# RicoFio/disentangle_mlp

Measured on AMD Instinct MI355X. Metric: celeba64_betavaegan_train_images_per_sec, higher is better.
Workload: dtype fp32-equivalent (fp16x3 split of fp32 operands on the f16 MFMA, fp32 accumulate, every convolution and the Linear layers with >= 2^20 weights (vg_gemm_nt_f16x3); the small Linear layers (vendor GEMMs), BatchNorm, losses, Adam in fp32)

## Files before the change

### disentangle_mlp_amd/_lib.py

```python
import ctypes
import os
from ctypes import c_float, c_int, c_size_t, c_void_p

import torch

_HERE = os.path.dirname(os.path.abspath(__file__))
LIB_PATH = os.path.join(_HERE, "libvaegan_hip.so")
ABI_VERSION = 7

_P, _I, _F, _Z = c_void_p, c_int, c_float, c_size_t

SIGNATURES = {
    "vg_version": (_I, []),
    "vg_conv5x5_fwd": (_I, [_P, _P, _P, _P, _I, _I, _I, _I, _I, _I, _P]),
    "vg_convT5x5_fwd": (_I, [_P, _P, _P, _P, _I, _I, _I, _I, _I, _I, _P]),
    "vg_conv5x5_packed_floats": (_Z, [_I, _I]),
    "vg_conv5x5_pack": (_I, [_P, _P, _I, _I, _I, _I, _P]),
    "vg_conv5x5_fwd_packed": (_I, [_P, _P, _P, _P, _I, _I, _I, _I, _I, _I, _P]),
    "vg_convT5x5_fwd_packed": (_I, [_P, _P, _P, _P, _I, _I, _I, _I, _I, _I, _P]),
    "vg_conv5x5_fwd_packed_stats_floats": (_Z, [_I, _I, _I, _I, _I, _I]),
    "vg_conv5x5_fwd_packed_stats": (_I, [_P, _P, _P, _P, _I, _I, _I, _I, _I, _I, _P, _Z, _P]),
    "vg_conv5x5_packed_bf16split_bytes": (_Z, [_I, _I, _I]),
    "vg_conv5x5_pack_bf16split": (_I, [_P, _P, _I, _I, _I, _I, _I, _P, _P]),
    "vg_gemm_nt_f16x3_workspace_bytes": (_Z, [_I, _I, _I]),
# ... 6 lines not shown
    "vg_conv_general_pack": (_I, [_P, _P, _I, _I, _I, _I, _P, _P]),
    "vg_conv_general_fwd": (_I, [_P, _P, _P, _P] + [_I] * 11 + [ctypes.c_long, _I, _P, _P, _P]),
    "vg_absmax": (_I, [_P, _Z, _P, _P]),
    "vg_absmax_affine": (_I, [_P, _P, _P, _I, _I, _I, _I, _P, _P]),
    "vg_absmax_multi": (_I, [_P, _I, _P]),
    "vg_conv5x5_pack_bf16split_multi": (_I, [_P, _I, _I, _P]),
    "vg_convT5x5_fwd_bf16split_workspace_bytes": (_Z, [_I, _I, _I, _I, _I, _I, _I]),
    "vg_convT5x5_fwd_bf16split": (_I, [_P, _P, _P, _P, _I, _I, _I, _I, _I, _I, _I, _P, _Z, _P, _P]),
    "vg_conv5x5_fwd_bf16split_workspace_bytes": (_Z, [_I, _I, _I, _I, _I, _I, _I]),
    "vg_conv5x5_bf16split_fusable": (_I, [_I, _I, _I, _I]),
    "vg_conv5x5_fwd_bf16split_stats_floats": (_Z, [_I, _I, _I, _I, _I, _I, _I]),
    "vg_convT5x5_fwd_bf16split_stats_floats": (_Z, [_I, _I, _I, _I, _I, _I, _I]),
    "vg_convT5x5_s1_thin_bf16split_ok": (_I, [_I, _I, _I, _I]),
    "vg_conv5x5_thin_wgrad_bf16split_workspace_bytes": (_Z, [_I, _I, _I, _I, _I, _I, _I]),
    "vg_conv5x5_thin_wgrad_bf16split": (_I, [_P, _P, _P, _I, _I, _I, _I, _I, _I, _I, _P, _Z, _P, _P, _I, _I, _P]),
    "vg_conv5x5_thin_bf16split_ok": (_I, [_I, _I, _I, _I, _I]),
    "vg_conv5x5_thin_bf16split_stats_floats": (_Z, [_I, _I, _I, _I, _I, _I]),
    "vg_conv5x5_thin_bf16split": (_I, [_P, _P, _P, _P, _I, _I, _I, _I, _I, _I, _I, _P, _Z, _P]),
    "vg_convT5x5_s1_thin_bf16split": (_I, [_P, _P, _P, _P, _I, _I, _I, _I, _I, _I, _P, _P, _I, _P]),
    "vg_conv5x5_fwd_bf16split": (_I, [_P, _P, _P, _P, _I, _I, _I, _I, _I, _I, _I, _P, _Z, _P, _P]),
    "vg_conv5x5_wgrad_bf16split_workspace_bytes": (_Z, [_I, _I, _I, _I, _I, _I, _I]),
    "vg_conv5x5_wgrad_bf16split": (_I, [_P, _P, _P, _I, _I, _I, _I, _I, _I, _I, _P, _Z, _P, _P, _I, _I, _P, _P, _I, _P]),
    "vg_conv5x5_wgrad_workspace_bytes": (_Z, [_I, _I, _I, _I, _I, _I]),
    "vg_conv5x5_wgrad": (_I, [_P, _P, _P, _I, _I, _I, _I, _I, _I, _P, _Z, _I, _P]),
    "vg_channel_sum": (_I, [_P, _P, _I, _I, _I, _P, _Z, _P]),
    "vg_bn_workspace_bytes": (_Z, [_I]),
    "vg_bn_act_fwd": (_I, [_P, _P, _P, _P, _P, _P, _P, _P, _I, _I, _I, _F, _F, _I, _P, _P, _Z, _P]),
    "vg_bn_act_bwd": (_I, [_P, _P, _P, _P, _P, _P, _P, _P, _P, _I, _I, _I, _I, _I, _P, _P, _Z, _P]),
    "vg_bn_finalize_stats": (_I, [_P, _I, _I, ctypes.c_double, _P, _P, _P, _P, _P, _P, _P, _P, _F, _F, _P, _P, _Z, _P]),
    "vg_bn_stats": (_I, [_P, _P, _P, _P, _P, _P, _P, _P, _P, _I, _I, _I, _F, _F, _P, _P, _Z, _P]),
    "vg_affine_act": (_I, [_P, _P, _P, _P, _I, _I, _I, _I, _P, _P]),
    "vg_bn_eval_coeffs": (_I, [_P, _P, _P, _P, _P, _P, _P, _I, _F, _I, _P, _I, ctypes.c_double, _P, _P]),
    "vg_bn_eval_act_bwd": (_I, [_P, _P, _P, _P, _P, _P, _P, _P, _P, _I, _I, _I, _I, _I, _P, _P, _Z, _P]),
    "vg_bias_act_fwd": (_I, [_P, _P, _P, _I, _I, _I, _I, _P]),
    "vg_act_bwd": (_I, [_P, _P, _P, _Z, _I, _P, _P]),
    "vg_reparam_kl_fwd": (_I, [_P, _P, _P, _P, _P, _P, _I, _I, _F, _P]),
    "vg_reparam_kl_bwd": (_I, [_P, _P, _P, _P, _P, _F, _P, _P, _I, _I, _P]),
    "vg_scale_by_scalar": (_I, [_P, _P, _P, _Z, _P]),
    "vg_sqdiff_workspace_bytes": (_Z, [_Z]),
    "vg_sqdiff_loss": (_I, [_P, _P, _P, _P, _Z, _F, _F, _P, _Z, _P]),
    "vg_bce_loss": (_I, [_P, _F, _P, _P, _I, _F, _F, _P]),
    "vg_adam_step": (_I, [_P, _I] + [ctypes.c_double] * 6 + [_P]),
    "vg_adam_prepare": (_I, [ctypes.c_double, _P, _I, ctypes.c_double, ctypes.c_double, ctypes.c_double, _P, _P]),
    "vg_adam_step_dev": (_I, [_P, _I] + [ctypes.c_double] * 3 + [_P, _P]),
    "vg_adam_step_checked": (_I, [_P, _I] + [ctypes.c_double] * 6 + [_P, _P]),
    "vg_adam_step_dev_checked": (_I, [_P, _I] + [ctypes.c_double] * 3 + [_P, _P, _P]),
    "vg_adam_step_ema": (_I, [_P, _I] + [ctypes.c_double] * 6 + [_P, _P, ctypes.c_double, _P]),
    "vg_adam_step_dev_ema": (_I, [_P, _I] + [ctypes.c_double] * 3 + [_P, _P, _P, ctypes.c_double, _P]),
    "vg_grad_sumsq_partials": (_Z, [_P, _I]),
    "vg_grad_sumsq_multi": (_I, [_P, _P, _I, _P, _Z, _P]),
    "vg_grad_clip_finalize": (_I, [_P, _Z, ctypes.c_double, _I, _P, _P]),
    "vg_adam_step_clip": (_I, [_P, _I] + [ctypes.c_double] * 6 + [_P, _P, ctypes.c_double, _P, _P]),
    "vg_adam_step_dev_clip": (_I, [_P, _I] + [ctypes.c_double] * 3 + [_P, _P, _P, ctypes.c_double, _P, _P]),
    "vg_adam_prepare_dev": (_I, [ctypes.c_double, _P, _I, _P, _I, ctypes.c_double, ctypes.c_double, _P, _P]),
    "vg_adam_step_decay": (_I, [_P, _I] + [ctypes.c_double] * 6 + [_P, _P, ctypes.c_double, _P, ctypes.c_double, _I, _P]),
    "vg_adam_step_dev_decay": (_I, [_P, _I] + [ctypes.c_double] * 3 + [_P, _P, _P, ctypes.c_double, _P, _P]),
    "vg_adam_step_dev_ema_dev": (_I, [_P, _I] + [ctypes.c_double] * 3 + [_P, _P, _P, _P, _P, _P]),
    "vg_reparam_kl_fwd_dev": (_I, [_P, _P, _P, _P, _P, _P, _I, _I, _P, _P]),
    "vg_reparam_kl_bwd_dev": (_I, [_P, _P, _P, _P, _P, _P, _P, _P, _I, _I, _P]),
    "vg_bce_loss_dev": (_I, [_P, _P, _P, _P, _I, _F, _F, _P]),
    "vg_dot_sigmoid_bce_workspace_bytes": (_Z, [_I]),
    "vg_dot_sigmoid_bce_fwd": (_I, [_P, _P, _P, _F, _P, _P, _P, _P, _I, _I, _F, _P, _Z, _P]),
    "vg_dot_sigmoid_bce_bwd": (_I, [_P, _P, _P, _P, _P, _P, _P, _I, _I, _I, _P]),
    "vg_u8_gather_normalize": (_I, [_P, _P, _P, _I, _I, _I, _I, _F, _F, _P]),
    "vg_minmax_workspace_bytes": (_Z, [_Z]),
    "vg_minmax": (_I, [_P, _Z, _P, _P, _Z, _P]),
    "vg_image_grid_shape": (_I, [_I, _I, _I, _I, _I, _P, _P]),
    "vg_image_grid_u8": (_I, [_P, _P, _P, _I, _I, _I, _I, _I, _I, _F, _P]),
    "vg_quantize_each_u8": (_I, [_P, _P, _I, _I, _I, _I, _P, _Z, _P]),
    "vg_resize_bilinear_u8": (_I, [_P, _P, _I, _I, _I, _I, _I, _F, _F, _P, _P]),
    "vg_pool3x3": (_I, [_P, _P] + [_I] * 9 + [_P, _P]),
    "vg_global_avg_pool": (_I, [_P, _P, _I, _I, _I, _P]),
}

TUNING_LIB_PATH = os.path.join(_HERE, "libvaegan_hip_tuning.so")
TUNING_SIGNATURES = {
    "vg_debug_set_conv_tile": (_I, [_I, _I]),
    "vg_debug_set_wgrad": (_I, [_I, _I]),
    "vg_debug_wgrad_plan": (_I, [_I, _I, _I, _I, _I, _I, _P, _P, _P, _P]),
    "vg_debug_wgrad_split_plan": (_I, [_I, _I, _I, _I, _I, _I, _I, _P]),
    "vg_debug_wgrad_thin_plan": (_I, [_I, _I, _I, _I, _I, _I, _I, _P, _P, _P]),
    "vg_debug_set_conv_bf16split_tile": (_I, [_I]),
    "vg_debug_set_conv_ring_tile": (_I, [_I]),
}

_lib = None
_product = None
_tuning = None


def _open(path, signatures):
    if not os.path.exists(path):
        raise ImportError(
            f"{path} not found: build it with `python -m disentangle_mlp_amd.build` "
            "(hipcc --offload-arch=gfx950). disentangle_mlp_amd has no CPU fallback.")
    lib = ctypes.CDLL(path)
    for name, (res, args) in signatures.items():
        fn = getattr(lib, name)
        fn.restype = res
        fn.argtypes = args
    built = lib.vg_version()
    if built != ABI_VERSION:
        raise ImportError(f"{path} was built for ABI {built}, this package binds ABI {ABI_VERSION}: rebuild it with "
                          "`python -m disentangle_mlp_amd.build`")
    return lib


def load():
    global _lib, _product
    if _lib is not None:
        return _lib
    if _product is None:
        _product = _open(LIB_PATH, SIGNATURES)
    _lib = _product
    return _lib


def load_tuning():
    global _tuning
    if _tuning is None:
        _tuning = _open(TUNING_LIB_PATH, {**SIGNATURES, **TUNING_SIGNATURES})
    return _tuning


class use_tuning:

    def __enter__(self):
        global _lib
        self._prev = load()
        _lib = load_tuning()
        return _lib

    def __exit__(self, *exc):
        global _lib
        _lib = self._prev
        return False


class ConvFusion(ctypes.Structure):
    _fields_ = [("in_scale", c_void_p), ("in_shift", c_void_p), ("in_act", c_int), ("stats", c_void_p),
                ("stats_floats", c_size_t), ("in_amax", c_void_p)]


class PackEntry(ctypes.Structure):
    _fields_ = [("w", c_void_p), ("packed", c_void_p), ("Cout", c_int), ("Cin", c_int), ("transposed", c_int),
                ("stride", c_int), ("w_amax", c_void_p)]


class AbsmaxEntry(ctypes.Structure):
    _fields_ = [("x", c_void_p), ("n", c_size_t), ("amax", c_void_p)]


class HipKernelError(RuntimeError):
    pass


def check(status, name):
    if status != 0:
        what = {-1: "bad argument", -2: "workspace too small"}.get(status, f"hipError_t {status}")
        raise HipKernelError(f"{name} failed: {what}")
```

### disentangle_mlp_amd/csrc/bn.hip

```cpp
#include "common.hpp"
#include "vaegan_hip.h"

namespace {

constexpr int NT = 256;
constexpr int NS_MAX = 64;

__device__ __forceinline__ float act_fwd(float v, int act) {
  if (act == VG_ACT_RELU) return v <= 0.f ? 0.f : v;
  if (act == VG_ACT_LRELU) return v > 0.f ? v : 0.2f * v;
  return v;
}
__device__ __forceinline__ float act_grad(float pre, float g, int act) {
  if (act == VG_ACT_RELU) return pre > 0.f ? g : 0.f;
  if (act == VG_ACT_LRELU) return pre > 0.f ? g : 0.2f * g;
  return g;
}

struct Slicing {
  int ns;
  long per;
};
Slicing make_slicing(int B, int C, int HW) {
  const long total = (long)B * HW;
  long ns = 2048 / C;
  if (ns < 1) ns = 1;
  if (ns > NS_MAX) ns = NS_MAX;
  long per = (total + ns - 1) / ns;
  if (per < 1024) per = 1024;
  per = (per + 3) / 4 * 4;
  ns = (total + per - 1) / per;
  Slicing s;
  s.ns = (int)ns;
  s.per = per;
  return s;
}

template <int MODE>
__global__ __launch_bounds__(NT) void bn_partial_kernel(const float* __restrict__ x, const float* __restrict__ gy,
                                                        const float* __restrict__ gamma,
                                                        const float* __restrict__ beta,
                                                        const float* __restrict__ mean,
                                                        const float* __restrict__ invstd, double* __restrict__ part,
                                                        int B, int C, int HW, long per, int ns, int act, int vec) {
  __shared__ double red[NT / 64];
  const int c = blockIdx.x, k = blockIdx.y;
  const long total = (long)B * HW;
  const long v0 = (long)k * per, v1 = min(v0 + per, total);
  const int hw_shift = (HW & (HW - 1)) == 0 ? __builtin_ctz(HW) : -1;
  double s1 = 0.0, s2 = 0.0;
  float mu = 0.f, is = 0.f, sc = 0.f, sh = 0.f;
  if (MODE == 1) {
    mu = mean[c];
    is = invstd[c];
    sc = gamma[c] * is;
    sh = beta[c] - mu * sc;
  }
  auto accum = [&](float xv, float gv) {
    if (MODE == 0) {
      s1 += xv;
      s2 += (double)xv * xv;
    } else if (MODE == 2) {
      s1 += xv;
    } else {
      const float g = act_grad(fmaf(xv, sc, sh), gv, act);
      s1 += g;
      s2 += (double)(g * ((xv - mu) * is));
    }
  };
  if (vec) {
    for (long v = v0 + 4L * threadIdx.x; v < v1; v += 4L * NT) {
      const long b = hw_shift >= 0 ? (v >> hw_shift) : v / HW, hw = v - b * HW;
      const size_t off = ((size_t)b * C + c) * HW + hw;
      const float4 xv = *reinterpret_cast<const float4*>(x + off);
      float4 gv = make_float4(0.f, 0.f, 0.f, 0.f);
      if (MODE == 1) gv = *reinterpret_cast<const float4*>(gy + off);
      accum(xv.x, gv.x);
      accum(xv.y, gv.y);
      accum(xv.z, gv.z);
      accum(xv.w, gv.w);
    }
  } else {
// ... 116 lines not shown
    }
  } else {
    for (long v = v0 + threadIdx.x; v < v1; v += NT) {
      const long b = hw_shift >= 0 ? (v >> hw_shift) : v / HW, hw = v - b * HW;
      const size_t off = ((size_t)b * C + c) * HW + hw;
      out[off] = one(x[off], BWD ? gy[off] : 0.f);
    }
  }
  if (out_amax) block_amax_atomic<NT>(am, out_amax);
}

constexpr int ONE_NT = 1024;

template <int NV>
__global__ __launch_bounds__(ONE_NT) void bn_bwd_onepass_kernel(const float* __restrict__ x, const float* __restrict__ gy,
                                                                const float* __restrict__ gamma,
                                                                const float* __restrict__ beta,
                                                                const float* __restrict__ mean,
                                                                const float* __restrict__ invstd, float* __restrict__ gx,
                                                                float* __restrict__ dgamma, float* __restrict__ dbeta,
                                                                int B, int C, int HW, int act,
                                                                unsigned* __restrict__ gx_amax) {
  __shared__ double red[ONE_NT / 64];
  __shared__ float s_c[2];
  const bool accp = (act & 0x100) != 0;
  act &= 0xff;
  const int c = blockIdx.x;
  const int total = B * HW;
  const int hw_shift = (HW & (HW - 1)) == 0 ? __builtin_ctz(HW) : -1;
  const float mu = mean[c], is = invstd[c], sc = gamma[c] * is, sh = beta[c] - mu * sc;
  float4 xv[NV], gv[NV];
  size_t off[NV];
#pragma unroll
  for (int j = 0; j < NV; ++j) {
    const int v = (j * ONE_NT + (int)threadIdx.x) * 4;
    const int vc = min(v, total - 4);
    const int b = hw_shift >= 0 ? (vc >> hw_shift) : vc / HW, hw = vc - b * HW;
    off[j] = ((size_t)b * C + c) * HW + hw;
    xv[j] = *reinterpret_cast<const float4*>(x + off[j]);
    gv[j] = *reinterpret_cast<const float4*>(gy + off[j]);
  }
  double s1 = 0.0, s2 = 0.0;
#pragma unroll
  for (int j = 0; j < NV; ++j) {
    const bool ok = (j * ONE_NT + (int)threadIdx.x) * 4 < total;
    float* xp = reinterpret_cast<float*>(&xv[j]);
    float* gp = reinterpret_cast<float*>(&gv[j]);
#pragma unroll
    for (int e = 0; e < 4; ++e) {
      const float g = ok ? act_grad(fmaf(xp[e], sc, sh), gp[e], act) : 0.f;
      gp[e] = g;
      s1 += g;
      s2 += (double)(g * ((xp[e] - mu) * is));
    }
  }
  const double t1 = block_sum<ONE_NT>(s1, red);
  const double t2 = block_sum<ONE_NT>(s2, red);
  if (threadIdx.x == 0) {
    const double count = (double)total;
    s_c[0] = (float)(t1 / count);
    s_c[1] = (float)(t2 / count);
    if (dbeta) dbeta[c] = (float)t1 + (accp ? dbeta[c] : 0.f);
    if (dgamma) dgamma[c] = (float)t2 + (accp ? dgamma[c] : 0.f);
  }
  __syncthreads();
  const float c1 = s_c[0], c2 = s_c[1];
  unsigned am = 0;
#pragma unroll
  for (int j = 0; j < NV; ++j) {
    if ((j * ONE_NT + (int)threadIdx.x) * 4 >= total) continue;
    const float* xp = reinterpret_cast<const float*>(&xv[j]);
    const float* gp = reinterpret_cast<const float*>(&gv[j]);
    float4 o;
    o.x = sc * (gp[0] - c1 - ((xp[0] - mu) * is) * c2);
    o.y = sc * (gp[1] - c1 - ((xp[1] - mu) * is) * c2);
    o.z = sc * (gp[2] - c1 - ((xp[2] - mu) * is) * c2);
    o.w = sc * (gp[3] - c1 - ((xp[3] - mu) * is) * c2);
    am = max(max(am, abs_bits(o.x)), max(max(abs_bits(o.y), abs_bits(o.z)), abs_bits(o.w)));
    *reinterpret_cast<float4*>(gx + off[j]) = o;
  }
  if (gx_amax) block_amax_atomic<ONE_NT>(am, gx_amax);
}

constexpr int B1_CH = 32, B1_SL = 8;

__global__ __launch_bounds__(NT) void bn1d_fwd_kernel(const float* __restrict__ x, const float* __restrict__ gamma,
                                                      const float* __restrict__ beta, float* __restrict__ y,
                                                      float* __restrict__ running_mean,
                                                      float* __restrict__ running_var, float* __restrict__ save_mean,
                                                      float* __restrict__ save_invstd, int B, int C, float eps,
                                                      float momentum, int act) {
  __shared__ double r1[B1_SL][B1_CH], r2[B1_SL][B1_CH];
  __shared__ float s_sc[B1_CH], s_sh[B1_CH];
  const int cl = threadIdx.x % B1_CH, sl = threadIdx.x / B1_CH;
  const int c = blockIdx.x * B1_CH + cl;
  const bool cok = c < C;
  double s1 = 0.0, s2 = 0.0;
  if (cok)
    for (int b = sl; b < B; b += B1_SL) {
      const float v = x[(size_t)b * C + c];
      s1 += v;
      s2 += (double)v * v;
    }
  r1[sl][cl] = s1;
  r2[sl][cl] = s2;
  __syncthreads();
  if (sl == 0 && cok) {
    double t1 = 0.0, t2 = 0.0;
#pragma unroll
    for (int k = 0; k < B1_SL; ++k) {
      t1 += r1[k][cl];
      t2 += r2[k][cl];
    }
    const double m = t1 / B;
    double var = t2 / B - m * m;
    if (var < 0.0) var = 0.0;
    const float mu = (float)m, is = (float)(1.0 / sqrt(var + (double)eps));
    save_mean[c] = mu;
    save_invstd[c] = is;
    if (running_mean) running_mean[c] = (1.f - momentum) * running_mean[c] + momentum * mu;
    if (running_var) {
      const double unb = B > 1 ? var * B / (B - 1.0) : var;
      running_var[c] = (1.f - momentum) * running_var[c] + momentum * (float)unb;
    }
    const float sc = gamma[c] * is;
    s_sc[cl] = sc;
    s_sh[cl] = beta[c] - mu * sc;
  }
  __syncthreads();
  if (cok) {
    const float sc = s_sc[cl], sh = s_sh[cl];
    for (int b = sl; b < B; b += B1_SL) {
      const size_t o = (size_t)b * C + c;
      y[o] = act_fwd(fmaf(x[o], sc, sh), act);
    }
  }
}

__global__ __launch_bounds__(NT) void bn1d_bwd_kernel(const float* __restrict__ gy, const float* __restrict__ x,
                                                      const float* __restrict__ gamma,
                                                      const float* __restrict__ beta,
                                                      const float* __restrict__ mean,
                                                      const float* __restrict__ invstd, float* __restrict__ gx,
                                                      float* __restrict__ dgamma, float* __restrict__ dbeta, int B,
                                                      int C, int act, unsigned* __restrict__ gx_amax) {
  const bool accp = (act & 0x100) != 0;
  act &= 0xff;
  __shared__ double r1[B1_SL][B1_CH], r2[B1_SL][B1_CH];
  __shared__ float s_c1[B1_CH], s_c2[B1_CH];
  const int cl = threadIdx.x % B1_CH, sl = threadIdx.x / B1_CH;
  const int c = blockIdx.x * B1_CH + cl;
  const bool cok = c < C;
  float mu = 0.f, is = 0.f, sc = 0.f, sh = 0.f;
  double s1 = 0.0, s2 = 0.0;
  if (cok) {
    mu = mean[c];
    is = invstd[c];
    sc = gamma[c] * is;
    sh = beta[c] - mu * sc;
    for (int b = sl; b < B; b += B1_SL) {
      const size_t o = (size_t)b * C + c;
      const float xv = x[o];
      const float g = act_grad(fmaf(xv, sc, sh), gy[o], act);
      s1 += g;
      s2 += (double)(g * ((xv - mu) * is));
    }
  }
  r1[sl][cl] = s1;
  r2[sl][cl] = s2;
  __syncthreads();
  if (sl == 0 && cok) {
    double t1 = 0.0, t2 = 0.0;
#pragma unroll
    for (int k = 0; k < B1_SL; ++k) {
      t1 += r1[k][cl];
      t2 += r2[k][cl];
    }
    if (dbeta) dbeta[c] = (float)t1 + (accp ? dbeta[c] : 0.f);
    if (dgamma) dgamma[c] = (float)t2 + (accp ? dgamma[c] : 0.f);
    s_c1[cl] = (float)(t1 / B);
    s_c2[cl] = (float)(t2 / B);
  }
  __syncthreads();
  unsigned am = 0;
  if (cok) {
    const float c1 = s_c1[cl], c2 = s_c2[cl];
    for (int b = sl; b < B; b += B1_SL) {
      const size_t o = (size_t)b * C + c;
      const float xv = x[o];
      const float g = act_grad(fmaf(xv, sc, sh), gy[o], act);
      const float r = sc * (g - c1 - ((xv - mu) * is) * c2);
      am = max(am, abs_bits(r));
      gx[o] = r;
    }
  }
  if (gx_amax) block_amax_atomic<NT>(am, gx_amax);
}

Slicing make_apply_slicing(int B, int C, int HW) {
  const long total = (long)B * HW;
  long ns = 4096 / C;
  if (ns < 1) ns = 1;
  long per = (total + ns - 1) / ns;
  if (per < 4096) per = 4096;
  per = (per + 3) / 4 * 4;
  Slicing s;
  s.per = per;
  s.ns = (int)((total + per - 1) / per);
  return s;
}

int streams_vec(int HW, const void* a, const void* b = nullptr, const void* c = nullptr) {
  return (HW & 3) == 0 && (((uintptr_t)a | (uintptr_t)b | (uintptr_t)c) & 15) == 0;
}

size_t part_bytes(int C) { return (size_t)C * NS_MAX * 2 * sizeof(double); }
size_t ws_bytes(int C) { return part_bytes(C) + 64; }

__device__ __forceinline__ float bn_act_bound(double s2, double m, double var, double count, double delta, float mu,
                                              float sc, float beta) {
  const double q = s2 / count;
  const double var_up = var + (3.01 * delta + 0x1p-50) * q;
  const double dev = sqrt(var_up * fmax(count - 1.0, 0.0)) + 1.01 * delta * sqrt(q) + 0x1p-23 * fabs(m);
  const double asc = fabs((double)sc), ab = fabs((double)beta);
  const double b = asc * dev + ab + 0x1p-23 * (ab + asc * fabs((double)mu));
  return (float)(b * (1.0 + 0x1p-20));
}

double slot_sums_delta(int nslots) { return (VG_STATS_SLOT_DEPTH + 1) * 0x1p-24 + (nslots + 2.0 * NS_MAX) * 0x1p-53; }

double fp64_sums_delta(double count) { return (count + 2.0 * NS_MAX + NT) * 0x1p-53; }

}

template <typename T>
__global__ __launch_bounds__(NT) void bn_finalize_kernel(const T* __restrict__ part, int np, long cs, long ks, int C,
                                                         double count, const float* __restrict__ gamma,
                                                         const float* __restrict__ beta, float* __restrict__ running_mean,
                                                         float* __restrict__ running_var, float* __restrict__ mean_out,
                                                         float* __restrict__ invstd_out, float* __restrict__ scale,
                                                         float* __restrict__ shift, float eps, float momentum,
                                                         unsigned* __restrict__ act_amax, double delta) {
  constexpr int CH = 32, KL = NT / CH;
  __shared__ double r1[KL][CH], r2[KL][CH];
  const int cl = threadIdx.x % CH, kl = threadIdx.x / CH;
  const int c = blockIdx.x * CH + cl;
  double s1 = 0.0, s2 = 0.0;
  if (c < C)
    for (int k = kl; k < np; k += KL) {
      s1 += (double)part[((size_t)c * cs + (size_t)k * ks) * 2];
      s2 += (double)part[((size_t)c * cs + (size_t)k * ks) * 2 + 1];
    }
  r1[kl][cl] = s1;
  r2[kl][cl] = s2;
  __syncthreads();
  if (kl == 0 && c < C) {
    s1 = 0.0;
    s2 = 0.0;
#pragma unroll
    for (int k = 0; k < KL; ++k) {
      s1 += r1[k][cl];
      s2 += r2[k][cl];
    }
    const double m = s1 / count;
    double var = s2 / count - m * m;
    if (var < 0.0) var = 0.0;
    const float mu = (float)m, is = (float)(1.0 / sqrt(var + (double)eps));
    const float sc = gamma[c] * is;
    mean_out[c] = mu;
    invstd_out[c] = is;
    scale[c] = sc;
    shift[c] = beta[c] - mu * sc;
    if (act_amax) atomicMax(act_amax, __float_as_uint(bn_act_bound(s2, m, var, count, delta, mu, sc, beta[c])));
    if (running_mean) running_mean[c] = (1.f - momentum) * running_mean[c] + momentum * mu;
    if (running_var) {
      const double unb = count > 1.0 ? var * count / (count - 1.0) : var;
      running_var[c] = (1.f - momentum) * running_var[c] + momentum * (float)unb;
    }
  }
}

__global__ __launch_bounds__(1024) void bn_finalize_wide_kernel(const float* __restrict__ stats, int nslots, int C,
                                                                double count, const float* __restrict__ gamma,
                                                                const float* __restrict__ beta,
                                                                float* __restrict__ running_mean,
                                                                float* __restrict__ running_var, float* __restrict__ mean_out,
                                                                float* __restrict__ invstd_out, float* __restrict__ scale,
                                                                float* __restrict__ shift, float eps, float momentum,
                                                                unsigned* __restrict__ act_amax, double delta) {
  constexpr int CH = 8, KL = 128;
  __shared__ double r1[KL][CH], r2[KL][CH];
  const int cl = threadIdx.x % CH, kl = threadIdx.x / CH;
  const int c = blockIdx.x * CH + cl;
  double s1 = 0.0, s2 = 0.0;
  if (c < C)
    for (int k = kl; k < nslots; k += KL) {
      const float2 v = *reinterpret_cast<const float2*>(stats + ((size_t)k * C + c) * 2);
      s1 += (double)v.x;
      s2 += (double)v.y;
    }
// ... 166 lines not shown
                     streams_vec(HW, x));
  VG_CHECK_LAUNCH();
  hipLaunchKernelGGL(bn_finalize_kernel<double>, dim3(cdiv(C, 32)), dim3(NT), 0, st, (const double*)part, s.ns,
                     (long)s.ns, 1L, C, (double)B * HW, gamma, beta, running_mean, running_var, save_mean, save_invstd,
                     scale, shift, eps, momentum, (unsigned*)act_amax, fp64_sums_delta((double)B * HW));
  VG_CHECK_LAUNCH();
  return 0;
}

extern "C" int vg_affine_act(const float* x, const float* scale, const float* shift, float* y, int B, int C, int HW,
                             int act, float* y_amax, void* stream) {
  if (!x || !scale || !shift || !y || B <= 0 || C <= 0 || HW <= 0) return VG_ERR_BAD_ARG;
  if (act < VG_ACT_NONE || act > VG_ACT_LRELU) return VG_ERR_BAD_ARG;
  if ((HW & 3) || (((uintptr_t)x | (uintptr_t)y) & 15)) {
    const size_t n = (size_t)B * C * HW;
    if (cdiv((long)n, (long)NT) > 0x7fffffffL) return VG_ERR_BAD_ARG;
    hipLaunchKernelGGL(affine_act_scalar_kernel, dim3((unsigned)((n + NT - 1) / NT)), dim3(NT), 0, (hipStream_t)stream, x,
                       scale, shift, y, C, HW, n, act, (unsigned*)y_amax);
    VG_CHECK_LAUNCH();
    return 0;
  }
  const size_t n4 = (size_t)B * C * HW / 4;
  if (cdiv((long)n4, (long)NT) > 0x7fffffffL) return VG_ERR_BAD_ARG;
  const int hw4 = HW / 4;
  int sh = -1;
  if ((hw4 & (hw4 - 1)) == 0 && n4 < (1ULL << 40)) {
    sh = 0;
    while ((1 << sh) < hw4) ++sh;
    if ((n4 >> sh) > 0xffffffffULL) sh = -1;
  }
  const size_t chunks = (n4 + NT * AA_U - 1) / (NT * AA_U);
  hipLaunchKernelGGL(affine_act_kernel, dim3((unsigned)(chunks < 2048 ? chunks : 2048)), dim3(NT), 0, (hipStream_t)stream, x, scale,
                     shift, y, C, HW, n4, act, sh, (unsigned*)y_amax);
  VG_CHECK_LAUNCH();
  return 0;
}

extern "C" int vg_bn_act_fwd(const float* x, const float* gamma, const float* beta, float* y, float* running_mean,
                             float* running_var, float* save_mean, float* save_invstd, int B, int C, int HW,
                             float eps, float momentum, int act, float* y_amax, void* workspace,
                             size_t workspace_bytes, void* stream) {
  if (!x || !gamma || !beta || !y || !save_mean || !save_invstd || B <= 0 || C <= 0 || HW <= 0)
    return VG_ERR_BAD_ARG;
  if (act < VG_ACT_NONE || act > VG_ACT_LRELU) return VG_ERR_BAD_ARG;
  hipStream_t st = (hipStream_t)stream;
  if (HW == 1) {
    hipLaunchKernelGGL(bn1d_fwd_kernel, dim3(cdiv(C, B1_CH)), dim3(NT), 0, st, x, gamma, beta, y, running_mean,
                       running_var, save_mean, save_invstd, B, C, eps, momentum, act);
    VG_CHECK_LAUNCH();
    return 0;
  }
  if (!workspace || workspace_bytes < ws_bytes(C)) return VG_ERR_WORKSPACE;
  double* part = (double*)workspace;
  const int vec = streams_vec(HW, x, y);
  const Slicing s = make_slicing(B, C, HW);
  hipLaunchKernelGGL(bn_partial_kernel<0>, dim3(C, s.ns), dim3(NT), 0, st, x, (const float*)nullptr, gamma, beta,
                     (const float*)nullptr, (const float*)nullptr, part, B, C, HW, s.per, s.ns, act, vec);
  VG_CHECK_LAUNCH();
  const Slicing a = make_apply_slicing(B, C, HW);
  hipLaunchKernelGGL(bn_apply_kernel<false>, dim3(C, a.ns), dim3(NT), 0, st, x, (const float*)nullptr,
                     (const double*)part, s.ns, gamma, beta, save_mean, save_invstd, running_mean, running_var,
                     (float*)nullptr, (float*)nullptr, y, B, C, HW, a.per, eps, momentum, act,
                     reinterpret_cast<unsigned*>(y_amax), vec);
  VG_CHECK_LAUNCH();
  return 0;
}

extern "C" int vg_bn_act_bwd(const float* gy, const float* x, const float* gamma, const float* beta,
                             const float* save_mean, const float* save_invstd, float* gx, float* dgamma,
                             float* dbeta, int B, int C, int HW, int act, int accumulate_param_grads, float* gx_amax,
                             void* workspace, size_t workspace_bytes, void* stream) {
  unsigned* am = (unsigned*)gx_amax;
  if (!gy || !x || !gamma || !beta || !save_mean || !save_invstd || !gx || B <= 0 || C <= 0 || HW <= 0)
    return VG_ERR_BAD_ARG;
  if (act < VG_ACT_NONE || act > VG_ACT_LRELU) return VG_ERR_BAD_ARG;
  hipStream_t st = (hipStream_t)stream;
  const int act_apply = act | (accumulate_param_grads ? 0x100 : 0);
  if (HW == 1) {
    hipLaunchKernelGGL(bn1d_bwd_kernel, dim3(cdiv(C, B1_CH)), dim3(NT), 0, st, gy, x, gamma, beta, save_mean,
                       save_invstd, gx, dgamma, dbeta, B, C, act_apply, am);
    VG_CHECK_LAUNCH();
    return 0;
  }
  const long per_channel = (long)B * HW;
  const int vec = streams_vec(HW, x, gy, gx);
  if (vec && per_channel >= 4 && per_channel <= (long)ONE_NT * 4 * 8 && C >= 128) {
    if (per_channel <= (long)ONE_NT * 4 * 2)
      hipLaunchKernelGGL(bn_bwd_onepass_kernel<2>, dim3(C), dim3(ONE_NT), 0, st, x, gy, gamma, beta, save_mean, save_invstd,
                         gx, dgamma, dbeta, B, C, HW, act_apply, am);
    else
      hipLaunchKernelGGL(bn_bwd_onepass_kernel<8>, dim3(C), dim3(ONE_NT), 0, st, x, gy, gamma, beta, save_mean, save_invstd,
                         gx, dgamma, dbeta, B, C, HW, act_apply, am);
    VG_CHECK_LAUNCH();
    return 0;
  }
  if (!workspace || workspace_bytes < ws_bytes(C)) return VG_ERR_WORKSPACE;
  double* part = (double*)workspace;
  const Slicing s = make_slicing(B, C, HW);
  hipLaunchKernelGGL(bn_partial_kernel<1>, dim3(C, s.ns), dim3(NT), 0, st, x, gy, gamma, beta, save_mean,
                     save_invstd, part, B, C, HW, s.per, s.ns, act, vec);
  VG_CHECK_LAUNCH();
  const Slicing a = make_apply_slicing(B, C, HW);
  hipLaunchKernelGGL(bn_apply_kernel<true>, dim3(C, a.ns), dim3(NT), 0, st, x, gy, (const double*)part, s.ns, gamma,
                     beta, const_cast<float*>(save_mean), const_cast<float*>(save_invstd), (float*)nullptr,
                     (float*)nullptr, dgamma, dbeta, gx, B, C, HW, a.per, 0.f, 0.f, act_apply, am, vec);
  VG_CHECK_LAUNCH();
  return 0;
}

namespace {

template <int CH, int KL>
__global__ __launch_bounds__(CH * KL) void bn_eval_coeffs_kernel(const float* __restrict__ gamma,
                                                                 const float* __restrict__ beta,
                                                                 const float* __restrict__ running_mean,
                                                                 const float* __restrict__ running_var,
                                                                 float* __restrict__ scale, float* __restrict__ shift,
                                                                 float* __restrict__ invstd, int C, float eps,
                                                                 const float* __restrict__ stats, int nslots, double count,
                                                                 unsigned* __restrict__ act_amax, double delta) {
  __shared__ double r1[KL][CH], r2[KL][CH];
  const int cl = threadIdx.x % CH, kl = threadIdx.x / CH;
  const int c = blockIdx.x * CH + cl;
  const bool bound = stats != nullptr && act_amax != nullptr;
  if (bound) {
    double s1 = 0.0, s2 = 0.0;
    if (c < C)
      for (int k = kl; k < nslots; k += KL) {
        s1 += (double)stats[((size_t)k * C + c) * 2];
        s2 += (double)stats[((size_t)k * C + c) * 2 + 1];
      }
    r1[kl][cl] = s1;
    r2[kl][cl] = s2;
    __syncthreads();
  }
  if (kl != 0 || c >= C) return;
  const float is = (float)(1.0 / sqrt((double)running_var[c] + (double)eps));
  const float sc = gamma[c] * is;
  const float sh = beta[c] - running_mean[c] * sc;
  scale[c] = sc;
  shift[c] = sh;
  invstd[c] = is;
  if (!bound) return;
  double s1 = 0.0, s2 = 0.0;
  for (int k = 0; k < KL; ++k) {
    s1 += r1[k][cl];
    s2 += r2[k][cl];
  }
  const double m = s1 / count, q = s2 / count;
  double var = q - m * m;
  if (var < 0.0) var = 0.0;
  const double var_up = var + (3.01 * delta + 0x1p-50) * q;
  const double dev = sqrt(var_up * fmax(count - 1.0, 0.0)) + 1.01 * delta * sqrt(q);
  const double asc = fabs((double)sc);
  const double b = asc * dev + fabs((double)sc * m + (double)sh) + 0x1p-21 * (asc * fabs(m) + fabs((double)sh));
  atomicMax(act_amax, __float_as_uint((float)(b * (1.0 + 0x1p-20))));
}

__device__ __forceinline__ float act_slope_of(int act) { return act == VG_ACT_RELU ? 0.f : act == VG_ACT_LRELU ? 0.2f : 1.f; }

__device__ __forceinline__ float eval_act_grad(float pre, float g, float slope) {
  const float d = pre > 0.f ? 1.f : slope;
  return (pre != pre && slope != 1.f) ? pre : g * d;
}

__global__ __launch_bounds__(NT) void bn_eval_bwd_kernel(const float* __restrict__ gy, const float* __restrict__ x,
                                                         const float* __restrict__ scale, const float* __restrict__ shift,
                                                         const float* __restrict__ mean, const float* __restrict__ invstd,
                                                         float* __restrict__ gx, double* __restrict__ part,
                                                         float* __restrict__ dgamma, float* __restrict__ dbeta, int B,
                                                         int C, int HW, long per, int ns, int act,
                                                         unsigned* __restrict__ gx_amax, int vec) {
  __shared__ double red[NT / 64];
  const bool accp = (act & 0x100) != 0;
  const float slope = act_slope_of(act & 0xff);
  const int c = blockIdx.x, k = blockIdx.y;
  const long total = (long)B * HW;
  const long v0 = (long)k * per, v1 = min(v0 + per, total);
  const int hw_shift = (HW & (HW - 1)) == 0 ? __builtin_ctz(HW) : -1;
  const float sc = scale[c], sh = shift[c], mu = mean[c], is = invstd[c];
  double s1 = 0.0, s2 = 0.0;
  unsigned am = 0;
  auto one = [&](float xv, float gv) -> float {
    const float g = eval_act_grad(fmaf(xv, sc, sh), gv, slope);
    s1 += g;
    s2 += (double)(g * ((xv - mu) * is));
    const float r = g * sc;
    am = max(am, abs_bits(r));
    return r;
  };
  if (vec) {
// ... 165 lines not shown
```

### include/vaegan_hip.h

```cpp
#ifndef VAEGAN_HIP_H
#define VAEGAN_HIP_H

#include <stddef.h>
#include <stdint.h>

#ifdef __cplusplus
extern "C" {
#endif

#define VG_ERR_BAD_ARG (-1)
#define VG_ERR_WORKSPACE (-2)

#define VG_ACT_NONE 0
#define VG_ACT_RELU 1
#define VG_ACT_LRELU 2

#define VG_ABI_VERSION 7
int vg_version(void);

int vg_conv5x5_fwd(const float* x, const float* w, const float* bias, float* y,
                   int B, int Cin, int H, int W, int Cout, int stride, void* stream);

int vg_convT5x5_fwd(const float* x, const float* w, const float* bias, float* y,
                    int B, int Cin, int H, int W, int Cout, int stride, void* stream);
// ... 167 lines not shown
  const float* g;
  float* m;
  float* v;
  size_t n;
  float* amax;
} VgAdamTensor;
int vg_adam_step(const VgAdamTensor* tensors, int count, double lr, double beta1, double beta2, double eps,
                 double bias_correction1, double bias_correction2_sqrt, void* stream);
int vg_adam_prepare(double step, double* step_dev, int advance_device_counter, double lr, double beta1, double beta2,
                    float* scalars, void* stream);
int vg_adam_step_dev(const VgAdamTensor* tensors, int count, double beta1, double beta2, double eps,
                     const float* scalars, void* stream);
#define VG_NONFINITE_GRAD 1u
#define VG_NONFINITE_PARAM 2u
int vg_adam_step_checked(const VgAdamTensor* tensors, int count, double lr, double beta1, double beta2, double eps,
                         double bias_correction1, double bias_correction2_sqrt, unsigned* const* nonfinite,
                         void* stream);
int vg_adam_step_dev_checked(const VgAdamTensor* tensors, int count, double beta1, double beta2, double eps,
                             const float* scalars, unsigned* const* nonfinite, void* stream);
int vg_adam_step_ema(const VgAdamTensor* tensors, int count, double lr, double beta1, double beta2, double eps,
                     double bias_correction1, double bias_correction2_sqrt, unsigned* const* nonfinite,
                     float* const* ema, double ema_decay, void* stream);
int vg_adam_step_dev_ema(const VgAdamTensor* tensors, int count, double beta1, double beta2, double eps,
                         const float* scalars, unsigned* const* nonfinite, float* const* ema, double ema_decay,
                         void* stream);
size_t vg_grad_sumsq_partials(const size_t* n, int count);
int vg_grad_sumsq_multi(const float* const* grads, const size_t* n, int count, double* partials, size_t capacity,
                        void* stream);
int vg_grad_clip_finalize(const double* partials, size_t n_partials, double max_norm, int skip_nonfinite, float* record,
                          void* stream);
int vg_adam_step_clip(const VgAdamTensor* tensors, int count, double lr, double beta1, double beta2, double eps,
                      double bias_correction1, double bias_correction2_sqrt, unsigned* const* nonfinite,
                      float* const* ema, double ema_decay, const float* clip_record, void* stream);
int vg_adam_step_dev_clip(const VgAdamTensor* tensors, int count, double beta1, double beta2, double eps,
                          const float* scalars, unsigned* const* nonfinite, float* const* ema, double ema_decay,
                          const float* clip_record, void* stream);
int vg_adam_prepare_dev(double step, double* step_dev, int advance_device_counter, const double* hyper, int decoupled,
                        double beta1, double beta2, float* scalars, void* stream);
int vg_adam_step_decay(const VgAdamTensor* tensors, int count, double lr, double beta1, double beta2, double eps,
                       double bias_correction1, double bias_correction2_sqrt, unsigned* const* nonfinite,
                       float* const* ema, double ema_decay, const float* clip_record, double weight_decay, int decoupled,
                       void* stream);
int vg_adam_step_dev_decay(const VgAdamTensor* tensors, int count, double beta1, double beta2, double eps,
                           const float* scalars, unsigned* const* nonfinite, float* const* ema, double ema_decay,
                           const float* clip_record, void* stream);
int vg_adam_step_dev_ema_dev(const VgAdamTensor* tensors, int count, double beta1, double beta2, double eps,
                             const float* scalars, unsigned* const* nonfinite, float* const* ema, const float* ema_omd,
                             const float* clip_record, void* stream);

int vg_u8_gather_normalize(const uint8_t* cache, const int64_t* index, float* out, int B, int C,
                           int H, int W, float mean, float stdv, void* stream);

size_t vg_minmax_workspace_bytes(size_t n);
int vg_minmax(const float* x, size_t n, float* out2, void* workspace, size_t workspace_bytes,
              void* stream);

int vg_image_grid_shape(int B, int H, int W, int nrow, int padding, int* grid_h, int* grid_w);
int vg_image_grid_u8(const float* x, const float* minmax, uint8_t* grid, int B, int C, int H, int W,
                     int nrow, int padding, float pad_value, void* stream);

int vg_quantize_each_u8(const float* x, uint8_t* out, int B, int C, int H, int W, void* workspace,
                        size_t workspace_bytes, void* stream);

int vg_resize_bilinear_u8(const uint8_t* img, float* y, int B, int H, int W, int OH, int OW, float scale, float shift,
                          float* amax, void* stream);

#define VG_POOL_MAX 0
#define VG_POOL_AVG_EXCLUDE_PAD 1
int vg_pool3x3(const float* x, float* out, int B, int C, int H, int W, int stride, int pad, int mode,
               int out_channels_total, int out_channel_offset, float* amax, void* stream);

int vg_global_avg_pool(const float* x, float* y, int B, int C, int HW, void* stream);

#ifdef VG_TUNING
int vg_debug_set_conv_tile(int mode, int variant);
int vg_debug_set_wgrad(int what, int value);
int vg_debug_wgrad_plan(int B, int Cin, int H, int W, int Cout, int stride, const void* gy, const void* dw,
                        const void* workspace, int* out);
int vg_debug_wgrad_split_plan(int B, int Cin, int H, int W, int Cout, int stride, int planes, int* out);
int vg_debug_wgrad_thin_plan(int B, int Cin, int H, int W, int Cout, int stride, int planes, const void* dw,
                             const void* workspace, int* out);
int vg_debug_set_conv_bf16split_tile(int variant);
int vg_debug_set_conv_ring_tile(int variant);
#endif

#ifdef __cplusplus
}
#endif
#endif
```

Measured before the change: 10100.

## Add team-based BN backward kernel with cross-workgroup spin exchange for large channels

Adds a batch-norm backward path for channels with many elements per channel. Teams of T workgroups split one channel, exchange partial double sums through tagged global-memory slots, and spin-wait on them, so a single kernel replaces the partial-sum and apply launches. Workgroups keep their x and gy values in registers across the exchange instead of reading them twice. The grid is capped at the CU count so all team members are co-resident. The cost is reliance on forward-progress assumptions, a spin timeout that writes NaN on failure, an extra zeroing launch, and a larger workspace.

Measured after the change: 10300 (median of 6 runs). 2.0% higher.

```diff
diff --git a/disentangle_mlp_amd/_lib.py b/disentangle_mlp_amd/_lib.py
--- a/disentangle_mlp_amd/_lib.py
+++ b/disentangle_mlp_amd/_lib.py
@@ -112,6 +112,8 @@
     "vg_debug_wgrad_thin_plan": (_I, [_I, _I, _I, _I, _I, _I, _I, _P, _P, _P]),
     "vg_debug_set_conv_bf16split_tile": (_I, [_I]),
     "vg_debug_set_conv_ring_tile": (_I, [_I]),
+    "vg_debug_set_bn_team": (_I, [_I, _I]),
+    "vg_debug_bn_bwd_plan": (_I, [_I, _I, _I, _P, _P, _P, _P]),
 }
 
 _lib = None
diff --git a/disentangle_mlp_amd/csrc/bn.hip b/disentangle_mlp_amd/csrc/bn.hip
--- a/disentangle_mlp_amd/csrc/bn.hip
+++ b/disentangle_mlp_amd/csrc/bn.hip
@@ -1,3 +1,5 @@
+#include <atomic>
+
 #include "common.hpp"
 #include "vaegan_hip.h"
 
@@ -280,6 +282,146 @@
   if (gx_amax) block_amax_atomic<ONE_NT>(am, gx_amax);
 }
 
+typedef __attribute__((address_space(1))) unsigned long long gu64;
+typedef __attribute__((address_space(1))) unsigned gu32;
+constexpr int TEAM_MAX_T = 16;
+constexpr int TEAM_MAX_WGS = 1024;
+constexpr size_t TEAM_HDR = 16;
+constexpr long long TEAM_SPIN_TICKS = 100000000;
+size_t team_block_bytes(int grid) { return TEAM_HDR + (size_t)grid * 2 * 4 * sizeof(unsigned long long); }
+
+__global__ __launch_bounds__(NT) void team_zero_kernel(unsigned long long* __restrict__ xch, int words) {
+  const int i = blockIdx.x * NT + threadIdx.x;
+  if (i < words) xch[i] = 0ull;
+}
+
+template <int NV>
+__global__ __launch_bounds__(ONE_NT) void bn_bwd_team_kernel(const float* __restrict__ x, const float* __restrict__ gy,
+                                                             const float* __restrict__ gamma,
+                                                             const float* __restrict__ beta,
+                                                             const float* __restrict__ mean,
+                                                             const float* __restrict__ invstd, float* __restrict__ gx,
+                                                             float* __restrict__ dgamma, float* __restrict__ dbeta, int B,
+                                                             int C, int HW, int act, unsigned* __restrict__ gx_amax, int T,
+                                                             int teams, unsigned long long* xch) {
+  __shared__ double red[ONE_NT / 64];
+  __shared__ float s_c[2];
+  __shared__ int s_failed;
+  const bool accp = (act & 0x100) != 0;
+  act &= 0xff;
+  const int team = blockIdx.x / T, member = blockIdx.x - team * T;
+  const int total = B * HW;
+  const int hw_shift = (HW & (HW - 1)) == 0 ? __builtin_ctz(HW) : -1;
+  const int v_base = member * (ONE_NT * 4 * NV);
+  gu32* status = (gu32*)xch;
+  gu64* sets = (gu64*)xch + TEAM_HDR / sizeof(unsigned long long) + (size_t)team * 2 * T * 4;
+  unsigned am = 0;
+  bool failed = false;
+  int round = 0;
+  for (int c = team; c < C; c += teams, ++round) {
+    const float mu = mean[c], is = invstd[c], sc = gamma[c] * is, sh = beta[c] - mu * sc;
+    float4 xv[NV], gv[NV];
+    auto offset_of = [&](int j) -> size_t {
+      const int v = v_base + (j * ONE_NT + (int)threadIdx.x) * 4;
+      const int vc = min(v, total - 4);
+      const int b = hw_shift >= 0 ? (vc >> hw_shift) : vc / HW, hw = vc - b * HW;
+      return ((size_t)b * C + c) * HW + hw;
+    };
+#pragma unroll
+    for (int j = 0; j < NV; ++j) {
+      const size_t off = offset_of(j);
+      xv[j] = *reinterpret_cast<const float4*>(x + off);
+      gv[j] = *reinterpret_cast<const float4*>(gy + off);
+    }
+    double s1 = 0.0, s2 = 0.0;
+#pragma unroll
+    for (int j = 0; j < NV; ++j) {
+      const bool ok = v_base + (j * ONE_NT + (int)threadIdx.x) * 4 < total;
+      float* xp = reinterpret_cast<float*>(&xv[j]);
+      float* gp = reinterpret_cast<float*>(&gv[j]);
+#pragma unroll
+      for (int e = 0; e < 4; ++e) {
+        const float g = ok ? act_grad(fmaf(xp[e], sc, sh), gp[e], act) : 0.f;
+        gp[e] = g;
+        s1 += g;
+        s2 += (double)(g * ((xp[e] - mu) * is));
+      }
+    }
+    const double t1 = block_sum<ONE_NT>(s1, red);
+    const double t2 = block_sum<ONE_NT>(s2, red);
+    if (threadIdx.x < 64) {
+      const int lane = threadIdx.x;
+      const unsigned tag = (unsigned)round + 1u;
+      gu64* set = sets + (size_t)(round & 1) * T * 4;
+      if (lane == 0) {
+        const unsigned long long b1 = (unsigned long long)__double_as_longlong(t1);
+        const unsigned long long b2 = (unsigned long long)__double_as_longlong(t2);
+        const unsigned long long hi = (unsigned long long)tag << 32;
+        gu64* mine = set + member * 4;
+        __hip_atomic_store(mine + 0, hi | (b1 & 0xffffffffull), __ATOMIC_RELAXED, __HIP_MEMORY_SCOPE_AGENT);
+        __hip_atomic_store(mine + 1, hi | (b1 >> 32), __ATOMIC_RELAXED, __HIP_MEMORY_SCOPE_AGENT);
+        __hip_atomic_store(mine + 2, hi | (b2 & 0xffffffffull), __ATOMIC_RELAXED, __HIP_MEMORY_SCOPE_AGENT);
+        __hip_atomic_store(mine + 3, hi | (b2 >> 32), __ATOMIC_RELAXED, __HIP_MEMORY_SCOPE_AGENT);
+      }
+      bool ok = false;
+      unsigned val = 0;
+      if (!failed) {
+        const bool has = lane < 4 * T;
+        const long long start = wall_clock64();
+        for (unsigned spins = 1;; ++spins) {
+          const unsigned long long g =
+              has ? __hip_atomic_load(set + lane, __ATOMIC_RELAXED, __HIP_MEMORY_SCOPE_AGENT) : (unsigned long long)tag << 32;
+          val = (unsigned)g;
+          if (__all((unsigned)(g >> 32) == tag)) {
+            ok = true;
+            break;
+          }
+          __builtin_amdgcn_s_sleep(2);
+          if ((spins & 63u) == 0 && __any(wall_clock64() - start > TEAM_SPIN_TICKS)) break;
+        }
+      }
+      double a1 = 0.0, a2 = 0.0;
+      for (int m = 0; m < T; ++m) {
+        const unsigned l1 = __shfl(val, 4 * m, 64), h1 = __shfl(val, 4 * m + 1, 64);
+        const unsigned l2 = __shfl(val, 4 * m + 2, 64), h2 = __shfl(val, 4 * m + 3, 64);
+        a1 += __longlong_as_double((long long)(((unsigned long long)h1 << 32) | l1));
+        a2 += __longlong_as_double((long long)(((unsigned long long)h2 << 32) | l2));
+      }
+      if (lane == 0) {
+        if (!ok) {
+          if (!failed) __hip_atomic_store(status, 1u, __ATOMIC_RELAXED, __HIP_MEMORY_SCOPE_AGENT);
+          a1 = a2 = __longlong_as_double(0x7ff8000000000000ll);
+        }
+        const double count = (double)total;
+        s_c[0] = (float)(a1 / count);
+        s_c[1] = (float)(a2 / count);
+        s_failed = !ok;
+        if (member == 0) {
+          if (dbeta) dbeta[c] = (float)a1 + (accp ? dbeta[c] : 0.f);
+          if (dgamma) dgamma[c] = (float)a2 + (accp ? dgamma[c] : 0.f);
+        }
+      }
+    }
+    __syncthreads();
+    const float c1 = s_c[0], c2 = s_c[1];
+    failed = s_failed != 0;
+#pragma unroll
+    for (int j = 0; j < NV; ++j) {
+      if (v_base + (j * ONE_NT + (int)threadIdx.x) * 4 >= total) continue;
+      const float* xp = reinterpret_cast<const float*>(&xv[j]);
+      const float* gp = reinterpret_cast<const float*>(&gv[j]);
+      float4 o;
+      o.x = sc * (gp[0] - c1 - ((xp[0] - mu) * is) * c2);
+      o.y = sc * (gp[1] - c1 - ((xp[1] - mu) * is) * c2);
+      o.z = sc * (gp[2] - c1 - ((xp[2] - mu) * is) * c2);
+      o.w = sc * (gp[3] - c1 - ((xp[3] - mu) * is) * c2);
+      am = max(max(am, abs_bits(o.x)), max(max(abs_bits(o.y), abs_bits(o.z)), abs_bits(o.w)));
+      *reinterpret_cast<float4*>(gx + offset_of(j)) = o;
+    }
+  }
+  if (gx_amax) block_amax_atomic<ONE_NT>(am, gx_amax);
+}
+
 constexpr int B1_CH = 32, B1_SL = 8;
 
 __global__ __launch_bounds__(NT) void bn1d_fwd_kernel(const float* __restrict__ x, const float* __restrict__ gamma,
@@ -413,7 +555,56 @@
 }
 
 size_t part_bytes(int C) { return (size_t)C * NS_MAX * 2 * sizeof(double); }
-size_t ws_bytes(int C) { return part_bytes(C) + 64; }
+size_t ws_bytes(int C) { return part_bytes(C) + 64 + team_block_bytes(TEAM_MAX_WGS); }
+
+int device_cus() {
+  constexpr int MAX_DEV = 64;
+  static std::atomic<int> cus[MAX_DEV];
+  int dev = 0;
+  if (hipGetDevice(&dev) != hipSuccess || dev < 0 || dev >= MAX_DEV) return 0;
+  int n = cus[dev].load(std::memory_order_relaxed);
+  if (n == 0) {
+    if (hipDeviceGetAttribute(&n, hipDeviceAttributeMultiprocessorCount, dev) != hipSuccess || n < 0) n = 0;
+    cus[dev].store(n, std::memory_order_relaxed);
+  }
+  return n;
+}
+
+VG_KNOB(int, g_team_nv, 0);
+VG_KNOB(int, g_team_max_wgs, 0);
+
+enum { BWD_1D = 0, BWD_ONE2 = 1, BWD_ONE8 = 2, BWD_TWO = 3, BWD_TEAM = 4 };
+struct BwdPlan {
+  int path, nv, T, teams, rounds;
+};
+BwdPlan make_bwd_plan(int B, int C, int HW, int vec) {
+  BwdPlan p = {BWD_TWO, 0, 0, 0, 0};
+  if (HW == 1) {
+    p.path = BWD_1D;
+    return p;
+  }
+  const long per_channel = (long)B * HW;
+  const bool forced = g_team_nv != 0;
+  if (!forced && vec && per_channel >= 4 && per_channel <= (long)ONE_NT * 4 * 8 && C >= 128) {
+    p.path = per_channel <= (long)ONE_NT * 4 * 2 ? BWD_ONE2 : BWD_ONE8;
+    return p;
+  }
+  if (!vec || per_channel < 4 || (!forced && per_channel <= (long)ONE_NT * 4 * 8)) return p;
+  const int nv = forced ? g_team_nv : 8;
+  const long cap = (long)ONE_NT * 4 * nv;
+  const long T = (per_channel + cap - 1) / cap;
+  if (T > TEAM_MAX_T || (!forced && (long)C * T < 128)) return p;
+  int max_wgs = device_cus();
+  if (g_team_max_wgs > 0 && g_team_max_wgs < max_wgs) max_wgs = g_team_max_wgs;
+  if (max_wgs > TEAM_MAX_WGS) max_wgs = TEAM_MAX_WGS;
+  if (max_wgs < T) return p;
+  p.path = BWD_TEAM;
+  p.nv = nv;
+  p.T = (int)T;
+  p.teams = (int)(C < max_wgs / T ? C : max_wgs / T);
+  p.rounds = (C + p.teams - 1) / p.teams;
+  return p;
+}
 
 __device__ __forceinline__ float bn_act_bound(double s2, double m, double var, double count, double delta, float mu,
                                               float sc, float beta) {
@@ -746,10 +937,31 @@
     VG_CHECK_LAUNCH();
     return 0;
   }
-  const long per_channel = (long)B * HW;
   const int vec = streams_vec(HW, x, gy, gx);
-  if (vec && per_channel >= 4 && per_channel <= (long)ONE_NT * 4 * 8 && C >= 128) {
-    if (per_channel <= (long)ONE_NT * 4 * 2)
+  const BwdPlan plan = make_bwd_plan(B, C, HW, vec);
+  if (plan.path == BWD_TEAM) {
+    const int grid = plan.teams * plan.T;
+    const size_t xbytes = team_block_bytes(grid);
+    if (!workspace || workspace_bytes < xbytes || ((uintptr_t)workspace & 15)) return VG_ERR_WORKSPACE;
+    unsigned long long* xch = (unsigned long long*)workspace;
+    const int words = (int)(xbytes / sizeof(unsigned long long));
+    hipLaunchKernelGGL(team_zero_kernel, dim3(cdiv(words, NT)), dim3(NT), 0, st, xch, words);
+    VG_CHECK_LAUNCH();
+    if (plan.nv == 8)
+      hipLaunchKernelGGL(bn_bwd_team_kernel<8>, dim3(grid), dim3(ONE_NT), 0, st, x, gy, gamma, beta, save_mean, save_invstd,
+                         gx, dgamma, dbeta, B, C, HW, act_apply, am, plan.T, plan.teams, xch);
+#ifdef VG_TUNING
+    else if (plan.nv == 1)
+      hipLaunchKernelGGL(bn_bwd_team_kernel<1>, dim3(grid), dim3(ONE_NT), 0, st, x, gy, gamma, beta, save_mean, save_invstd,
+                         gx, dgamma, dbeta, B, C, HW, act_apply, am, plan.T, plan.teams, xch);
+#endif
+    else
+      return VG_ERR_BAD_ARG;
+    VG_CHECK_LAUNCH();
+    return 0;
+  }
+  if (plan.path == BWD_ONE2 || plan.path == BWD_ONE8) {
+    if (plan.path == BWD_ONE2)
       hipLaunchKernelGGL(bn_bwd_onepass_kernel<2>, dim3(C), dim3(ONE_NT), 0, st, x, gy, gamma, beta, save_mean, save_invstd,
                          gx, dgamma, dbeta, B, C, HW, act_apply, am);
     else
@@ -771,6 +983,22 @@
   VG_CHECK_LAUNCH();
   return 0;
 }
+
+#ifdef VG_TUNING
+extern "C" int vg_debug_set_bn_team(int nv, int max_wgs) {
+  if ((nv != 0 && nv != 1 && nv != 8) || max_wgs < 0) return VG_ERR_BAD_ARG;
+  g_team_nv = nv;
+  g_team_max_wgs = max_wgs;
+  return 0;
+}
+
+extern "C" int vg_debug_bn_bwd_plan(int B, int C, int HW, const void* gy, const void* x, const void* gx, int* out) {
+  if (!out || B <= 0 || C <= 0 || HW <= 0) return VG_ERR_BAD_ARG;
+  const BwdPlan p = make_bwd_plan(B, C, HW, streams_vec(HW, x, gy, gx));
+  out[0] = p.path; out[1] = p.nv; out[2] = p.T; out[3] = p.teams; out[4] = p.rounds;
+  return 0;
+}
+#endif
 
 namespace {
 
diff --git a/include/vaegan_hip.h b/include/vaegan_hip.h
--- a/include/vaegan_hip.h
+++ b/include/vaegan_hip.h
@@ -273,6 +273,8 @@
                              const void* workspace, int* out);
 int vg_debug_set_conv_bf16split_tile(int variant);
 int vg_debug_set_conv_ring_tile(int variant);
+int vg_debug_set_bn_team(int nv, int max_wgs);
+int vg_debug_bn_bwd_plan(int B, int C, int HW, const void* gy, const void* x, const void* gx, int* out);
 #endif
 
 #ifdef __cplusplus
```
